# HKU-MedAI/WSI-HGNN

Hardware: AMD Instinct MI355X
Metric: edges/s fwd+bwd HEATNet4, 10k-node/6-rel synth graph, 1->8 MI355X (higher is better)
Workload: dtype f32 (fp16x3 emulation: 2-way fp16 split scaled per row (Y = XW^T, dX) or per column (dW), 3 products - bf16x6 for small launches; fp32-class error)

## Files before the change

### include/wsi_hgnn.h

```cpp
#ifndef WSI_HGNN_H
#define WSI_HGNN_H

#include <stdint.h>

#ifdef __cplusplus
extern "C" {
#endif

#define WSI_OK        0
#define WSI_EINVAL  (-22)
#define WSI_ENOSYS  (-38)
#define WSI_EFAULT  (-14)
#define WSI_ENOMEM  (-12)

#define WSI_ABI_VERSION 26

int         wsi_abi_version(void);
const char* wsi_last_error(void);

typedef struct wsi_context wsi_context_t;
int  wsi_context_create(wsi_context_t** out);
void wsi_context_destroy(wsi_context_t* ctx);

#define WSI_ATTN_XCD_CONTIGUOUS 1
#define WSI_ATTN_HUB_DEGREE(d) (((d) & 0xffff) << 8)
int wsi_heat_attn_fwd(const float* q, int64_t ldq, const float* k, int64_t ldk, const float* v, int64_t ldv,
                      int32_t num_nodes, int32_t D, int32_t H,
                      const int32_t* node_seg, const int32_t* rowptr, const int32_t* src, const float* sim,
                      const int32_t* order, int32_t num_heavy, int32_t flags,
                      const float* e_weight, const float* e_bias,
                      float* t, int64_t ldt, float* score, float* lse,
                      uint32_t* t_absmax,
                      wsi_context_t* ctx, void* stream);

int wsi_heat_attn_scores_fwd(const float* q, int64_t ldq, const float* k, int64_t ldk, int32_t num_nodes, int32_t D, int32_t H,
                             const int32_t* node_seg, const int32_t* rowptr, const int32_t* src, const float* sim,
                             const int32_t* order, int32_t num_heavy, int32_t flags, const float* e_weight, const float* e_bias,
                             float* score, float* lse, wsi_context_t* ctx, void* stream);

int wsi_heat_pool_coeff(const float* score, const float* lse, const int32_t* edge_seg,
                        const int32_t* colptr, const int32_t* csc_eid, const int32_t* csc_dst, const float* inv_rd,
                        const int32_t* row_seg, int32_t segs_per_type, int32_t n_types, int32_t H, int32_t num_src,
                        float* ctab, void* stream);

int wsi_heat_pool_gtab(const float* h, int64_t ldh, int32_t D, int32_t H, const float* y, const float* beta,
                       const int32_t* chunk_row, const int32_t* chunk_seg, int32_t num_chunks,
                       int32_t segs_per_type, int32_t n_types, float* gtab, void* stream);

typedef struct wsi_attn_pool {
    const int32_t* row_seg;
    int32_t segs_per_type, n_types;
    const float* y;
    const float* g_row;
    const float* omg;
    float* r_out; int64_t ldr;
    float* ctab;
    int32_t ctab_ready;
    const float* h; int64_t ldh;
    const float* beta;
    const float* gtab;
    const int32_t* edge_seg;
    const int32_t* seg_dst;
} wsi_attn_pool_t;

int wsi_heat_attn_bwd(const float* q, int64_t ldq, const float* k, int64_t ldk, const float* v, int64_t ldv,
                      int32_t num_nodes, int32_t num_src, int32_t num_edges, int32_t D, int32_t H,
                      const int32_t* node_seg, const int32_t* rowptr, const int32_t* src, const float* sim,
                      const int32_t* colptr, const int32_t* csc_eid, const int32_t* csc_dst,
                      const float* inv_rd, const int32_t* order_dst, int32_t num_heavy, const int32_t* order_src, int32_t flags,
                      const float* e_weight, const float* e_bias,
                      const float* g_t, int64_t ldgt,
                      const int32_t* g_t_row,
                      const float* score,
                      float* score_a,
                      const float* lse,
                      float* ga, float* gsc, float* gea, float* red_ws,
                      float* gq, int64_t ldgq, float* gk, int64_t ldgk, float* gv, int64_t ldgv,
                      float* g_e,
                      uint32_t* g_absmax,
                      const wsi_attn_pool_t* pool,
                      wsi_context_t* ctx, void* stream);

typedef struct wsi_gemm_group {
    const float* A;
    const float* B;
    float*       C;
    const float* bias;
    const float* R;
    const float* gate;
    const float* B1;
    const float* B2;
    int64_t lda, ldb, ldc, ldr;
    int32_t M, N, K;
    int32_t b_chunk;
    const float* Mm;
    int64_t  ldm;
    float*   colsum_out;
    const uint32_t* a_absmax;
    uint32_t*       c_absmax;
    int32_t a_absmax_parts;
    int32_t c_absmax_parts;
    int32_t c_absmax_first;
    int32_t reserved;
    uint32_t drop_seed;
    uint32_t drop_threshold;
    float    drop_scale;
    int32_t  drop_row0;
    int32_t  drop_cols;
    int32_t  drop_col0;
    const uint32_t* drop_seed_base;
    uint32_t*       c_colmax;
    float*          c_colsum;
    int64_t         c_col_ld;
    const uint32_t* a_colmax;
    const float*    a_colsum;
    const uint32_t* b_colmax;
    int64_t         a_col_ld, b_col_ld;
    int32_t         a_col_parts, b_col_parts;
    void*           b_packed;
} wsi_gemm_group_t;

#define WSI_GEMM_NT 0
#define WSI_GEMM_NN 1
#define WSI_GEMM_TN 2

#define WSI_EPI_BIAS        1
#define WSI_EPI_ACCUMULATE  2
#define WSI_EPI_SCALE_GATE  4
#define WSI_EPI_GELU        8
#define WSI_EPI_ADD_R       16
// ... 222 lines not shown
```

### wsi-hgnn_amd/csrc/gemm_tn16.hip

```cpp
#include "gemm_common.h"
#include "emu16.h"

namespace wsi {

typedef __attribute__((__vector_size__(4 * sizeof(__fp16)))) __fp16 h16x4;
typedef __attribute__((address_space(3))) h16x4 lds_h16x4;
typedef _Float16 f16x4 __attribute__((ext_vector_type(4)));

constexpr int T_M = 256;
constexpr int T_THREADS = 512;
constexpr int T_KS = 16;
#ifndef T_NS_DEF
#define T_NS_DEF 3
#endif
constexpr int T_NS = T_NS_DEF;
constexpr int T_CH = 256;

struct TnGroup {
    const float* A; const float* B;
    const uint32_t* abits; const uint32_t* bbits;
    int64_t lda, ldb;
    int64_t ws_off;
    int32_t M, N, K;
    int32_t tile_start, tiles_n, tiles_mn, kchunk, flags;
};
struct TnParams {
    TnGroup g[WSI_GEMM_MAX_GROUPS];
    int32_t ngroups, total_tiles;
};

__device__ __forceinline__ f16x8 tr_read8(const uint16_t* p0, const uint16_t* p1) {
    const h16x4 lo = __builtin_amdgcn_ds_read_tr16_b64_v4f16((lds_h16x4*)p0);
    const h16x4 hi = __builtin_amdgcn_ds_read_tr16_b64_v4f16((lds_h16x4*)p1);
    const f16x4 a = __builtin_bit_cast(f16x4, lo), b = __builtin_bit_cast(f16x4, hi);
    return __builtin_shufflevector(a, b, 0, 1, 2, 3, 4, 5, 6, 7);
}

template <int TN_, int NACC>
__global__ __launch_bounds__(T_THREADS, 2) void gemm_tn16_kernel(const TnParams P, float* __restrict__ ws) {
    static_assert(TN_ == 128 || TN_ == 256, "tile width");
    constexpr int PA = T_M + 32, PB = TN_ + 32;
    constexpr int PLANE_A = T_KS * PA, PLANE_B = T_KS * PB;
    constexpr int BUF = 2 * (PLANE_A + PLANE_B);
    constexpr int CB = TN_ / 4;
    constexpr int NBQ = TN_ / 128;
    constexpr int RB = T_THREADS / CB;
    constexpr int WTN = TN_ / 64;
    __shared__ __attribute__((aligned(16))) uint16_t smem[2 * BUF];

    const int tid = threadIdx.x;
    const int tile = xcd_remap((int)blockIdx.x, P.total_tiles);
    int gi = 0;
#pragma unroll 1
    for (int i = 1; i < P.ngroups; ++i) gi = (tile >= P.g[i].tile_start) ? i : gi;
    const TnGroup& G = P.g[gi];
    int local = tile - G.tile_start;
    const int split = local / G.tiles_mn;
    local -= split * G.tiles_mn;
    const int tm = local / G.tiles_n, tn = local - tm * G.tiles_n;
    const int m0 = tm * T_M, n0 = tn * TN_;
    const int kb = split * G.kchunk, ke = min(G.K, kb + G.kchunk);
    const int lane = tid & 63, wave = tid >> 6;
    const int wm = wave >> 1, wn = wave & 1;
    const int l31 = lane & 31, hi = lane >> 5;

    const int c4a = tid & 63, ra = tid >> 6;
    const int c4b = tid % CB, rb = tid / CB;
    float sa[4], sb[4];
#pragma unroll
    for (int i = 0; i < 4; ++i) {
        sa[i] = __builtin_ldexpf(1.f, -scale_exponent(G.abits[min(m0 + 4 * c4a + i, G.M - 1)]));
        sb[i] = __builtin_ldexpf(1.f, -scale_exponent(G.bbits[min(n0 + 4 * c4b + i, G.N - 1)]));
    }
    const int wA = min(T_M, G.M - m0), wB = min(TN_, G.N - n0);
    const bool fast = (G.flags & 1) && (G.flags & 2) && (wA % 4 == 0) && (wB % 4 == 0) && ke > kb &&
                      (int64_t)(ke - kb) * G.lda * 4 < ((int64_t)1 << 31) && (int64_t)(ke - kb) * G.ldb * 4 < ((int64_t)1 << 31);
    typedef uint32_t u32x4 __attribute__((ext_vector_type(4)));
    const float* baseA = G.A + (int64_t)kb * G.lda + m0;
    const float* baseB = G.B + (int64_t)kb * G.ldb + n0;
    const auto rsA = __builtin_amdgcn_make_buffer_rsrc(const_cast<float*>(baseA), 0, fast ? (int)(((int64_t)(ke - kb - 1) * G.lda + wA) * 4) : 0, 0x00020000);
    const auto rsB = __builtin_amdgcn_make_buffer_rsrc(const_cast<float*>(baseB), 0, fast ? (int)(((int64_t)(ke - kb - 1) * G.ldb + wB) * 4) : 0, 0x00020000);
    const int voA = (int)((ra * G.lda + 4 * c4a) * 4), voB = (int)((rb * G.ldb + 4 * c4b) * 4);
    const int stepA = (int)(G.lda * 4), stepB = (int)(G.ldb * 4);
    struct Stage { float4 a[2]; float4 b[NBQ]; };
    auto as_f4 = [](const u32x4& v) { return make_float4(__uint_as_float(v[0]), __uint_as_float(v[1]), __uint_as_float(v[2]), __uint_as_float(v[3])); };
    auto load_fast = [&](Stage& S, int s) {
#pragma unroll
        for (int q = 0; q < 2; ++q) S.a[q] = as_f4(__builtin_amdgcn_raw_buffer_load_b128(rsA, voA, (s * T_KS + 8 * q) * stepA, 0));
#pragma unroll
        for (int q = 0; q < NBQ; ++q) S.b[q] = as_f4(__builtin_amdgcn_raw_buffer_load_b128(rsB, voB, (s * T_KS + RB * q) * stepB, 0));
    };
    auto load4g = [](const float* __restrict__ row, int c0, int c_end) {
        float4 r = make_float4(0.f, 0.f, 0.f, 0.f);
        if (c0 + 0 < c_end) r.x = row[c0 + 0];
        if (c0 + 1 < c_end) r.y = row[c0 + 1];
        if (c0 + 2 < c_end) r.z = row[c0 + 2];
        if (c0 + 3 < c_end) r.w = row[c0 + 3];
        return r;
    };
    auto load_guarded = [&](Stage& S, int k0) {
#pragma unroll
        for (int q = 0; q < 2; ++q) {
            const int k = k0 + ra + 8 * q;
            S.a[q] = (k < ke) ? load4g(G.A + (int64_t)k * G.lda, m0 + 4 * c4a, G.M) : make_float4(0.f, 0.f, 0.f, 0.f);
        }
#pragma unroll
        for (int q = 0; q < NBQ; ++q) {
            const int k = k0 + rb + RB * q;
            S.b[q] = (k < ke) ? load4g(G.B + (int64_t)k * G.ldb, n0 + 4 * c4b, G.N) : make_float4(0.f, 0.f, 0.f, 0.f);
        }
    };
    const int nfast = fast ? (ke - kb + T_KS - 1) / T_KS : 0;
// ... 50 lines not shown
#pragma unroll
        for (int i = 0; i < 2; ++i)
#pragma unroll
            for (int j = 0; j < WTN; ++j) c[i][j] = __builtin_amdgcn_mfma_f32_32x32x16_f16(a[i], b[j], c[i][j], 0, 0, 0);
    };
    constexpr int CX = NACC - 1;
    auto multiply_stage = [&](const uint16_t* buf) {
        f16x8 a0[2], a1[2], b0[WTN], b1[WTN];
        read_a(buf, 0, a0);
        read_b(buf, 1, b1);
        read_a(buf, 1, a1);
        read_b(buf, 0, b0);
        products(acc[CX], a0, b1);
        products(acc[CX], a1, b0);
        products(acc[0], a0, b0);
    };

    if (nfast > 0) {
        constexpr int NS = (TN_ == 128) ? T_NS : 2;
        Stage R[NS];
        struct Frags { f16x8 a0[2], a1[2], b0[WTN], b1[WTN]; };
        auto body = [&](Frags& c, Frags& n, Stage& C, Stage& F, int s) {
            load_fast(F, min(s + NS, nfast - 1));
            const uint16_t* cur = smem + (s & 1) * BUF;
            uint16_t* oth = smem + ((s + 1) & 1) * BUF;
            __builtin_amdgcn_s_setprio(2);
            read_a(cur, 1, c.a1);
            read_b(cur, 0, c.b0);
            products(acc[CX], c.a0, c.b1);
            store_stage(C, oth);
            products(acc[CX], c.a1, c.b0);
            __builtin_amdgcn_sched_group_barrier(0x020, 2 + NBQ, 0);
            __builtin_amdgcn_sched_group_barrier(0x100, 2 * (2 + WTN), 0);
#pragma unroll
            for (int m = 0; m < 4 * WTN; ++m) {
                __builtin_amdgcn_sched_group_barrier(0x008, 1, 0);
                __builtin_amdgcn_sched_group_barrier(0x002, 3, 0);
                if (m >= 4 * WTN - (2 + NBQ)) __builtin_amdgcn_sched_group_barrier(0x200, 2, 0);
            }
            __builtin_amdgcn_s_setprio(0);
            __builtin_amdgcn_sched_barrier(0);
            __syncthreads();
            read_a(oth, 0, n.a0);
            read_b(oth, 1, n.b1);
            products(acc[0], c.a0, c.b0);
            __builtin_amdgcn_sched_barrier(0);
        };
#pragma unroll
        for (int q = 0; q < NS; ++q) load_fast(R[q], min(q, nfast - 1));
        store_stage(R[0], smem);
        __syncthreads();
        Frags X, Y;
        read_a(smem, 0, X.a0);
        read_b(smem, 1, X.b1);
        int s = 0;
        for (; s + 2 * NS <= nfast; s += 2 * NS) {
#pragma unroll
            for (int q = 0; q < 2 * NS; ++q) {
                if (q & 1) body(Y, X, R[(q + 1) % NS], R[q % NS], s + q);
                else body(X, Y, R[(q + 1) % NS], R[q % NS], s + q);
            }
        }
#pragma unroll
        for (int q = 0; q < 2 * NS - 1; ++q) {
            if (s + q < nfast) {
                if (q & 1) body(Y, X, R[(q + 1) % NS], R[q % NS], s + q);
                else body(X, Y, R[(q + 1) % NS], R[q % NS], s + q);
            }
        }
    }
    for (int k0 = kb + nfast * T_KS; k0 < ke; k0 += T_KS) {
        Stage g;
        load_guarded(g, k0);
        store_stage(g, smem);
        __syncthreads();
        multiply_stage(smem);
        __syncthreads();
    }

    int* se = reinterpret_cast<int*>(smem);
    for (int i = tid; i < T_M + TN_; i += T_THREADS)
        se[i] = (i < T_M) ? scale_exponent(G.abits[min(m0 + i, G.M - 1)]) : scale_exponent(G.bbits[min(n0 + i - T_M, G.N - 1)]);
    __syncthreads();
    float* slab = ws + G.ws_off + (int64_t)split * G.M * G.N;
#pragma unroll
    for (int j = 0; j < WTN; ++j) {
        const int cl = wn * (TN_ / 2) + j * 32 + l31;
        const int col = n0 + cl;
        const int ec = se[T_M + cl];
#pragma unroll
        for (int i = 0; i < 2; ++i)
#pragma unroll
            for (int r = 0; r < 16; ++r) {
                const int rl = wm * 64 + i * 32 + (r & 3) + 8 * (r >> 2) + 4 * hi;
                const int row = m0 + rl;
                float x = acc[0][i][j][r];
                if constexpr (NACC == 2) x = fmaf(acc[1][i][j][r], 1.f / LO_SCALE, x);
                x = __builtin_ldexpf(x, ec + se[rl]);
                if (row < G.M && col < G.N) slab[(int64_t)row * G.N + col] = x;
            }
    }
}

struct ColJob {
    const float* X; int64_t ld;
    const uint32_t* part;
    const float* psum;
    int64_t part_ld;
    int32_t own;
    uint32_t* out;
    float* sum_out;
    const float* gate;
    int32_t rows, cols, cols_pad, chunks, col_blocks;
    int32_t block_start;
    int32_t fblock_start;
    int32_t vec;
};
struct ColParams {
    ColJob j[2 * WSI_GEMM_MAX_GROUPS];
    int32_t njobs, epilogue;
};

__global__ __launch_bounds__(256) void colstat_partial_kernel(const ColParams P) {
    __shared__ float4 sm[256], ss[256];
    int ji = 0;
#pragma unroll 1
    for (int i = 1; i < P.njobs; ++i) ji = (P.j[i].own && (int)blockIdx.x >= P.j[i].block_start) ? i : ji;
    const ColJob& J = P.j[ji];
    if (!J.own) return;
    const int b = (int)blockIdx.x - J.block_start;
    const int chunk = b / J.col_blocks, cb = b - chunk * J.col_blocks;
    const int c4 = threadIdx.x & 63, rl = threadIdx.x >> 6;
    const int c0 = cb * 256 + 4 * c4;
    const int r0 = chunk * T_CH, r1 = min(J.rows, r0 + T_CH);
    float4 m = make_float4(0.f, 0.f, 0.f, 0.f), t = make_float4(0.f, 0.f, 0.f, 0.f);
    if (J.vec && c0 + 3 < J.cols) {
        const float* p = J.X + c0;
#pragma unroll 4
        for (int r = r0 + rl; r < r1; r += 4) {
            const float4 v = *reinterpret_cast<const float4*>(p + (int64_t)r * J.ld);
            m.x = fmaxf(m.x, fabsf(v.x)); m.y = fmaxf(m.y, fabsf(v.y)); m.z = fmaxf(m.z, fabsf(v.z)); m.w = fmaxf(m.w, fabsf(v.w));
            t.x += v.x; t.y += v.y; t.z += v.z; t.w += v.w;
        }
    } else if (c0 < J.cols) {
        for (int r = r0 + rl; r < r1; r += 4) {
            const float* p = J.X + (int64_t)r * J.ld + c0;
            m.x = fmaxf(m.x, fabsf(p[0])); t.x += p[0];
            if (c0 + 1 < J.cols) { m.y = fmaxf(m.y, fabsf(p[1])); t.y += p[1]; }
            if (c0 + 2 < J.cols) { m.z = fmaxf(m.z, fabsf(p[2])); t.z += p[2]; }
            if (c0 + 3 < J.cols) { m.w = fmaxf(m.w, fabsf(p[3])); t.w += p[3]; }
        }
    }
    sm[threadIdx.x] = m;
    ss[threadIdx.x] = t;
    __syncthreads();
    if (rl == 0 && c0 < J.cols_pad) {
#pragma unroll
        for (int q = 1; q < 4; ++q) {
            const float4 o = sm[c4 + 64 * q], u = ss[c4 + 64 * q];
            m.x = fmaxf(m.x, o.x); m.y = fmaxf(m.y, o.y); m.z = fmaxf(m.z, o.z); m.w = fmaxf(m.w, o.w);
            t.x += u.x; t.y += u.y; t.z += u.z; t.w += u.w;
        }
        *reinterpret_cast<uint4*>(const_cast<uint32_t*>(J.part) + (int64_t)chunk * J.part_ld + c0) =
            make_uint4(__float_as_uint(m.x), __float_as_uint(m.y), __float_as_uint(m.z), __float_as_uint(m.w));
        if (J.psum) *reinterpret_cast<float4*>(const_cast<float*>(J.psum) + (int64_t)chunk * J.part_ld + c0) = t;
    }
}

constexpr int CF_COLS = 16, CF_LANES = 256 / CF_COLS;
__global__ __launch_bounds__(256) void colstat_final_kernel(const ColParams P) {
    __shared__ uint32_t sm[256];
    __shared__ float ss[256];
    int ji = 0;
#pragma unroll 1
    for (int i = 1; i < P.njobs; ++i) ji = ((int)blockIdx.x >= P.j[i].fblock_start) ? i : ji;
    const ColJob& J = P.j[ji];
    const int cl = threadIdx.x % CF_COLS, kl = threadIdx.x / CF_COLS;
    const int c = ((int)blockIdx.x - J.fblock_start) * CF_COLS + cl;
    uint32_t m = 0u;
    float t = 0.f;
    if (c < J.cols) {
        const uint32_t* pm = J.part + c;
// ... 31 lines not shown

static inline bool tn_vec_ok(const void* p, int64_t ld) { return ((reinterpret_cast<uintptr_t>(p) & 15) == 0) && (ld % 4 == 0); }

static int tn16_tile_n() {
    const char* s = knob("WSI_TN16_CFG");
    return (s && s[0] == '2') ? 256 : 128;
}

struct Tn16Plan {
    int32_t splits[WSI_GEMM_MAX_GROUPS];
    int32_t kchunk[WSI_GEMM_MAX_GROUPS];
    int32_t tiles_m[WSI_GEMM_MAX_GROUPS], tiles_n[WSI_GEMM_MAX_GROUPS];
    int32_t total_tiles;
};

static void tn16_plan(const wsi_gemm_group_t* g, int32_t ng, int tn, Tn16Plan& pl) {
    const int64_t target = 256;
    int64_t work = 0, maxk = 0;
    for (int i = 0; i < ng; ++i) {
        pl.tiles_m[i] = pl.tiles_n[i] = 0; pl.splits[i] = 1; pl.kchunk[i] = g[i].K > 0 ? g[i].K : T_KS;
        if (g[i].M <= 0 || g[i].N <= 0) continue;
        pl.tiles_m[i] = (g[i].M + T_M - 1) / T_M; pl.tiles_n[i] = (g[i].N + tn - 1) / tn;
        work += (int64_t)pl.tiles_m[i] * pl.tiles_n[i] * g[i].K;
        if (g[i].K > maxk) maxk = g[i].K;
    }
    int64_t kc = (work + target - 1) / target;
    kc = ((kc + T_KS - 1) / T_KS) * T_KS;
    if (kc < 8 * T_KS) kc = 8 * T_KS;
    for (;;) {
        int64_t blocks = 0;
        for (int i = 0; i < ng; ++i) {
            if (!pl.tiles_m[i]) continue;
            pl.splits[i] = g[i].K > 0 ? (int32_t)((g[i].K + kc - 1) / kc) : 1;
            blocks += (int64_t)pl.tiles_m[i] * pl.tiles_n[i] * pl.splits[i];
        }
        if (blocks <= target || kc >= maxk) break;
        kc += T_KS;
    }
    int32_t tiles = 0;
    for (int i = 0; i < ng; ++i) {
        if (!pl.tiles_m[i]) continue;
        if (g[i].K > 0) {
            int64_t per = (g[i].K + pl.splits[i] - 1) / pl.splits[i];
            per = ((per + T_KS - 1) / T_KS) * T_KS;
            pl.kchunk[i] = (int32_t)per;
            pl.splits[i] = (int32_t)((g[i].K + per - 1) / per);
        }
        tiles += pl.tiles_m[i] * pl.tiles_n[i] * pl.splits[i];
    }
    pl.total_tiles = tiles;
}

static inline int64_t pad4(int64_t x) { return (x + 3) & ~(int64_t)3; }

int64_t tn16_workspace_floats(const wsi_gemm_group_t* groups, int32_t ngroups) {
    Tn16Plan pl;
    tn16_plan(groups, ngroups, tn16_tile_n(), pl);
    int64_t f = 0;
    for (int i = 0; i < ngroups; ++i) {
        if (groups[i].M <= 0 || groups[i].N <= 0) continue;
        f += (int64_t)pl.splits[i] * groups[i].M * groups[i].N;
    }
    f = pad4(f);
    for (int i = 0; i < ngroups; ++i) {
        if (groups[i].M <= 0 || groups[i].N <= 0) continue;
        const int64_t chunks = (groups[i].K + T_CH - 1) / T_CH;
        f += (pad4(groups[i].M) + pad4(groups[i].N)) * (1 + chunks) + (groups[i].colsum_out ? pad4(groups[i].M) * chunks : 0);
    }
    return f;
}

int launch_gemm_tn16(int32_t epilogue, const wsi_gemm_group_t* groups, int32_t ngroups, float* ws, int64_t ws_bytes, hipStream_t st) {
    const int tn = tn16_tile_n();
    Tn16Plan pl;
    tn16_plan(groups, ngroups, tn, pl);
    const int64_t need = tn16_workspace_floats(groups, ngroups);
    if (need >= ((int64_t)1 << 31)) { set_error("gemm TN fp16x3: workspace of %lld floats exceeds the 2^31 index range", (long long)need); return WSI_EINVAL; }
    if (!ws || ws_bytes < need * 4) { set_error("gemm TN fp16x3: workspace of %lld bytes needed, %lld given", (long long)(need * 4), (long long)ws_bytes); return WSI_ENOMEM; }
    if (reinterpret_cast<uintptr_t>(ws) & 15) { set_error("gemm TN fp16x3: the workspace must be 16-byte aligned"); return WSI_EINVAL; }
    TnParams P;
    ReduceParams RP;
    ColParams CP;
    P.ngroups = 0; RP.ngroups = 0; RP.epilogue = epilogue; CP.njobs = 0;
    int64_t f = 0, red_total = 0;
    int32_t tiles = 0;
    for (int i = 0; i < ngroups; ++i) {
        const wsi_gemm_group_t& s = groups[i];
        if (s.M <= 0 || s.N <= 0) continue;
        TnGroup& d = P.g[P.ngroups];
        d.A = s.A; d.B = s.B; d.lda = s.lda; d.ldb = s.ldb; d.M = s.M; d.N = s.N; d.K = s.K;
        d.tiles_n = pl.tiles_n[i]; d.tiles_mn = pl.tiles_m[i] * pl.tiles_n[i]; d.kchunk = pl.kchunk[i];
        d.tile_start = tiles;
        tiles += d.tiles_mn * pl.splits[i];
        d.flags = (tn_vec_ok(s.A, s.lda) ? 1 : 0) | (tn_vec_ok(s.B, s.ldb) ? 2 : 0);
        d.ws_off = f;
        ReduceDesc& r = RP.g[RP.ngroups++];
        r.ws = ws + f; r.C = s.C; r.gate = s.gate; r.ldc = s.ldc; r.M = s.M; r.N = s.N; r.pad = 0; r.splits = pl.splits[i]; r.start = red_total;
        red_total += (int64_t)s.M * s.N;
        f += (int64_t)pl.splits[i] * s.M * s.N;
        r.cs_ws = nullptr; r.cs_out = nullptr;
        P.ngroups++;
    }
    if (P.ngroups == 0) return WSI_OK;
    P.total_tiles = tiles;
    f = pad4(f);
    uint32_t* wu = reinterpret_cast<uint32_t*>(ws);
    int32_t pblocks = 0, fblocks = 0;
    CP.epilogue = epilogue;
    auto job_for = [&](const float* X, int64_t ld, int32_t rows, int32_t cols, float* sum_out, const float* gate,
                       const uint32_t* gmax, const float* gsum, int64_t gld, int32_t gparts, int64_t& cursor) -> const uint32_t* {
        if (gmax && (gparts < 1 || (sum_out && !gsum))) gmax = nullptr;
        for (int q = 0; q < CP.njobs; ++q) {
            ColJob& J = CP.j[q];
            if (J.X == X && J.ld == ld && J.rows == rows && J.cols == cols && !sum_out && (J.own || J.part == gmax)) return J.out;
        }
        ColJob& J = CP.j[CP.njobs++];
        J.X = X; J.ld = ld; J.rows = rows; J.cols = cols; J.cols_pad = (int32_t)pad4(cols);
        J.col_blocks = (cols + 255) / 256;
        J.out = wu + cursor; cursor += J.cols_pad;
        J.sum_out = sum_out; J.gate = gate;
        if (gmax) {
            J.own = 0; J.part = gmax; J.psum = sum_out ? gsum : nullptr; J.part_ld = gld; J.chunks = gparts; J.vec = 0;
            J.block_start = pblocks;
        } else {
            J.own = 1; J.part_ld = J.cols_pad; J.chunks = (rows + T_CH - 1) / T_CH;
            J.part = wu + cursor; cursor += (int64_t)J.chunks * J.cols_pad;
            J.psum = nullptr;
            if (sum_out) { J.psum = reinterpret_cast<float*>(wu + cursor); cursor += (int64_t)J.chunks * J.cols_pad; }
            J.vec = tn_vec_ok(X, ld) ? 1 : 0;
            J.block_start = pblocks; pblocks += J.chunks * J.col_blocks;
        }
        J.fblock_start = fblocks; fblocks += (cols + CF_COLS - 1) / CF_COLS;
        return J.out;
    };
    {
        int gidx = 0;
        for (int i = 0; i < ngroups; ++i) {
            const wsi_gemm_group_t& s = groups[i];
            if (s.M <= 0 || s.N <= 0) continue;
            TnGroup& d = P.g[gidx++];
            int64_t cursor = f;
            d.abits = job_for(s.A, s.lda, s.K, s.M, s.colsum_out, s.gate, s.a_colmax, s.a_colsum, s.a_col_ld, s.a_col_parts, cursor);
            d.bbits = job_for(s.B, s.ldb, s.K, s.N, nullptr, nullptr, s.b_colmax, nullptr, s.b_col_ld, s.b_col_parts, cursor);
            const int64_t chunks = (s.K + T_CH - 1) / T_CH;
            f += (pad4(s.M) + pad4(s.N)) * (1 + chunks) + (s.colsum_out ? pad4(s.M) * chunks : 0);
        }
    }
    if (pblocks > 0) hipLaunchKernelGGL(colstat_partial_kernel, dim3(pblocks), dim3(256), 0, st, CP);
    hipLaunchKernelGGL(colstat_final_kernel, dim3(fblocks), dim3(256), 0, st, CP);
#ifdef WSI_ABLATE
    if (tn == 256) hipLaunchKernelGGL((gemm_tn16_kernel<256, 1>), dim3(tiles), dim3(T_THREADS), 0, st, P, ws);
    else
#endif
    hipLaunchKernelGGL((gemm_tn16_kernel<128, 2>), dim3(tiles), dim3(T_THREADS), 0, st, P, ws);
    RP.total = red_total;
    launch_splitk_reduce(RP, st);
    return check_launch("gemm_tn16");
}

}

using namespace wsi;

extern "C" int32_t wsi_col_stats_parts(int32_t rows) { return rows > 0 ? (rows + T_CH - 1) / T_CH : 0; }

extern "C" int wsi_col_stats(const float* x, int64_t ld, int32_t rows, int32_t cols, uint32_t* part_max, float* part_sum, int64_t part_ld, void* stream) {
    if (rows < 0 || cols < 0) { set_error("col_stats: bad shape %d x %d", rows, cols); return WSI_EINVAL; }
    if (rows == 0 || cols == 0) return WSI_OK;
    if (!x || !part_max || part_ld < ((cols + 3) & ~3) || (part_ld & 3) || (reinterpret_cast<uintptr_t>(part_max) & 15) || (part_sum && (reinterpret_cast<uintptr_t>(part_sum) & 15))) {
        set_error("col_stats: null pointer, or tables not 16-byte aligned with a pitch >= the columns rounded up to 4"); return WSI_EINVAL; }
    ColParams CP;
    CP.njobs = 1; CP.epilogue = 0;
    ColJob& J = CP.j[0];
    J.X = x; J.ld = ld; J.rows = rows; J.cols = cols; J.cols_pad = (int32_t)pad4(cols); J.col_blocks = (cols + 255) / 256;
    J.out = nullptr; J.sum_out = nullptr; J.gate = nullptr; J.own = 1; J.part_ld = part_ld; J.chunks = (rows + T_CH - 1) / T_CH;
    J.part = part_max; J.psum = part_sum; J.vec = tn_vec_ok(x, ld) ? 1 : 0;
    J.block_start = 0; J.fblock_start = 0;
    hipLaunchKernelGGL(colstat_partial_kernel, dim3(J.chunks * J.col_blocks), dim3(256), 0, (hipStream_t)stream, CP);
    return check_launch("col_stats");
}

extern "C" int64_t wsi_col_absmax_workspace_bytes(int32_t rows, int32_t cols) {
    if (rows <= 0 || cols <= 0) return 0;
    return (int64_t)((rows + T_CH - 1) / T_CH) * pad4(cols) * 4;
}

extern "C" int wsi_col_absmax(const float* x, int64_t ld, int32_t rows, int32_t cols, uint32_t* out, void* workspace, int64_t workspace_bytes, void* stream) {
    if (rows < 0 || cols < 0) { set_error("col_absmax: bad shape %d x %d", rows, cols); return WSI_EINVAL; }
    if (cols == 0) return WSI_OK;
    if (!out || (rows > 0 && !x)) { set_error("col_absmax: null pointer"); return WSI_EINVAL; }
    const int64_t need = wsi_col_absmax_workspace_bytes(rows, cols);
    if (need > 0 && (!workspace || workspace_bytes < need || (reinterpret_cast<uintptr_t>(workspace) & 15))) {
        set_error("col_absmax: a 16-byte aligned workspace of %lld bytes is needed", (long long)need); return WSI_ENOMEM; }
    ColParams CP;
    CP.njobs = 1; CP.epilogue = 0;
    ColJob& J = CP.j[0];
    J.X = x; J.ld = ld; J.rows = rows; J.cols = cols; J.cols_pad = (int32_t)pad4(cols); J.col_blocks = (cols + 255) / 256;
    J.out = out; J.sum_out = nullptr; J.gate = nullptr; J.own = 1; J.part_ld = J.cols_pad; J.chunks = (rows + T_CH - 1) / T_CH;
    J.part = reinterpret_cast<uint32_t*>(workspace); J.psum = nullptr; J.vec = tn_vec_ok(x, ld) ? 1 : 0;
    J.block_start = 0; J.fblock_start = 0;
    hipStream_t st = (hipStream_t)stream;
    if (J.chunks > 0) hipLaunchKernelGGL(colstat_partial_kernel, dim3(J.chunks * J.col_blocks), dim3(256), 0, st, CP);
    hipLaunchKernelGGL(colstat_final_kernel, dim3((cols + CF_COLS - 1) / CF_COLS), dim3(256), 0, st, CP);
    return check_launch("col_absmax");
}
```

### wsi-hgnn_amd/csrc/loss.hip

```cpp
#include "common.h"
#include <math.h>

namespace wsi {

constexpr int64_t CE_IGNORE_INDEX = -100;
__global__ __launch_bounds__(256) void cross_entropy_kernel(const float* __restrict__ logits, const int64_t* __restrict__ labels, int B, int C,
                                                            float* __restrict__ loss, float* __restrict__ dlogits, int* __restrict__ bad) {
    __shared__ float part[256];
    __shared__ int cnt[256];
    __shared__ int any_bad;
    if (threadIdx.x == 0) any_bad = 0;
    int valid = 0;
    for (int b = threadIdx.x; b < B; b += 256) {
        const int64_t y = labels[b];
        valid += (y >= 0 && y < C) ? 1 : 0;
    }
    cnt[threadIdx.x] = valid;
    __syncthreads();
    for (int o = 128; o > 0; o >>= 1) {
        if ((int)threadIdx.x < o) cnt[threadIdx.x] += cnt[threadIdx.x + o];
        __syncthreads();
    }
    const int nvalid = cnt[0];
    const float invB = nvalid > 0 ? 1.f / (float)nvalid : 0.f;
    float acc = 0.f;
    for (int b = threadIdx.x; b < B; b += 256) {
        const float* row = logits + (int64_t)b * C;
        const int64_t y = labels[b];
        if (y < 0 || y >= C) {
            if (y != CE_IGNORE_INDEX) { any_bad = 1; if (bad) *bad = 1; }
            for (int c = 0; c < C; ++c) dlogits[(int64_t)b * C + c] = 0.f;
            continue;
        }
        float mx = -INFINITY;
        for (int c = 0; c < C; ++c) mx = fmaxf(mx, row[c]);
        float den = 0.f;
        for (int c = 0; c < C; ++c) den += expf(row[c] - mx);
        acc += (logf(den) + mx) - row[y];
        const float inv = 1.f / den;
        for (int c = 0; c < C; ++c) dlogits[(int64_t)b * C + c] = (expf(row[c] - mx) * inv - (c == y ? 1.f : 0.f)) * invB;
    }
    part[threadIdx.x] = acc;
    __syncthreads();
    for (int o = 128; o > 0; o >>= 1) {
        if ((int)threadIdx.x < o) part[threadIdx.x] += part[threadIdx.x + o];
        __syncthreads();
    }
    if (threadIdx.x == 0) *loss = any_bad ? NAN : part[0] / (float)nvalid;
}

}

using namespace wsi;

extern "C" int wsi_cross_entropy(const float* logits, const int64_t* labels, int32_t B, int32_t C, float* loss, float* dlogits, int32_t* bad_label,
                                 void* stream) {
    if (B <= 0 || C <= 0 || (int64_t)B * C > 65536) { set_error("cross_entropy: unsupported shape %d x %d", B, C); return WSI_ENOSYS; }
    if (!logits || !labels || !loss || !dlogits) { set_error("cross_entropy: null pointer"); return WSI_EINVAL; }
    hipLaunchKernelGGL(cross_entropy_kernel, dim3(1), dim3(256), 0, (hipStream_t)stream, logits, labels, (int)B, (int)C, loss, dlogits, (int*)bad_label);
    return check_launch("cross_entropy");
}
```

### wsi-hgnn_amd/ops.py

```python
from __future__ import annotations

import ctypes
import contextlib
from typing import List, Optional, Sequence, Tuple

import torch

from . import _native as N
from .graph import GraphPlan, SegmentTable, host_to_device



_TIMING = {"on": False, "records": []}


def enable_kernel_timing(on: bool) -> None:
    _TIMING["on"] = bool(on)
    _TIMING["records"] = []


class _Timed:
    def __init__(self, name: str, flops: float = 0.0, mfma_flops: float = 0.0):
        self.name, self.flops, self.mfma_flops = name, flops, mfma_flops

# ... 196 lines not shown
        st = _SIDE_STREAMS["streams"][key] = torch.cuda.Stream(device=dev)
    return st


def _side_stats_on() -> bool:
    return _SIDE_STATS["enabled"] and not _SIDE_STATS["reasons"] and not torch.cuda.is_current_stream_capturing()


def block_side_streams(blocked: bool, who: str) -> None:
    (_SIDE_STATS["reasons"].add if blocked else _SIDE_STATS["reasons"].discard)(who)
    block_background_weight_gradients(blocked, who=who)


def set_side_column_statistics(on: bool) -> None:
    _SIDE_STATS["enabled"] = bool(on)


def _col_stats_side(x: torch.Tensor, rows: Sequence[Tuple[int, int]], device):
    if not _side_stats_on():
        return None
    lib = N.load()
    dev = torch.device(device)
    width = x.shape[1]
    wpad = (width + 3) & ~3
    ranges, p = {}, 0
    for (a, b) in rows:
        if (a, b) not in ranges and b > a:
            n_ = lib.wsi_col_stats_parts(b - a)
            ranges[(a, b)] = (p, n_)
            p += n_
    if p == 0:
        return None
    bits = torch.empty((p, wpad), dtype=torch.int32, device=dev)
    sums = torch.empty((p, wpad), dtype=torch.float32, device=dev)
    side = side_stream(dev, "stats")
    main = torch.cuda.current_stream(dev)
    side.wait_stream(main)
    for (a, b), (p0, n_) in ranges.items():
        N.check(lib.wsi_col_stats(N.ptr(x, a * x.stride(0) * 4), x.stride(0), b - a, width, N.ptr(bits, p0 * wpad * 4), N.ptr(sums, p0 * wpad * 4), wpad,
                                  ctypes.c_void_p(side.cuda_stream)), "wsi_col_stats")
        _SIDE_STATS["launches"] += 1
    ev = torch.cuda.Event()
    ev.record(side)
    for t_ in (x, bits, sums):
        t_.record_stream(side)
    return ColStats(bits, sums, ranges), ev


def remember_constant_cols(x: torch.Tensor, rows: Sequence[Tuple[int, int]]) -> None:
    if _PRECISION["mode"] not in _SCALED_MODES or x.dim() != 2 or not x.is_cuda or x.stride(1) != 1:
        return
    st = _annotation(x, "_wsi_col_stats")
    if st is not None and all(r in st.ranges for r in rows if r[1] > r[0]):
        return
    lib = N.load()
    width = x.shape[1]
    ranges, bits_rows = {}, []
    for (a, b) in rows:
        if (a, b) in ranges or b <= a:
            continue
        out = torch.empty(width, dtype=torch.int32, device=x.device)
        nbytes = lib.wsi_col_absmax_workspace_bytes(b - a, width)
        ws = torch.empty(max(nbytes // 4, 4), dtype=torch.int32, device=x.device)
        N.check(lib.wsi_col_absmax(N.ptr(x, a * x.stride(0) * 4), x.stride(0), b - a, width, N.ptr(out), N.ptr(ws), nbytes, N.stream()), "wsi_col_absmax")
        ranges[(a, b)] = (len(bits_rows), 1)
        bits_rows.append(out)
    if bits_rows:
        attach_col_stats(x, ColStats(torch.stack(bits_rows), None, ranges))


def refresh_constant_cols(x: torch.Tensor) -> None:
    st = _annotation(x, "_wsi_col_stats")
    if st is None or st.sums is not None:
        return
    lib = N.load()
    width = x.shape[1]
    for (a, b), (p0, _) in st.ranges.items():
        nbytes = lib.wsi_col_absmax_workspace_bytes(b - a, width)
        ws = torch.empty(max(nbytes // 4, 4), dtype=torch.int32, device=x.device)
        N.check(lib.wsi_col_absmax(N.ptr(x, a * x.stride(0) * 4), x.stride(0), b - a, width, N.ptr(st.bits, p0 * st.bits.shape[1] * 4), N.ptr(ws), nbytes,
                                   N.stream()), "wsi_col_absmax")


_PACKED = {"enabled": True, "entries": {}, "hits": 0, "packs": 0}


def set_packed_weight_cache(on: bool) -> None:
    _PACKED["enabled"] = bool(on)
    if not on:
        _PACKED["entries"].clear()


def invalidate_packed_weights() -> None:
    _PACKED["entries"].clear()


def _pack_groups(op: int, items, arm: bool) -> None:
    lib = N.load()
    for i in range(0, len(items), N.WSI_GEMM_MAX_GROUPS):
        chunk = items[i:i + N.WSI_GEMM_MAX_GROUPS]
        arr = _group_array([g for _, g in chunk])
        N.check(lib.wsi_gemm_pack_b(op, arr, len(chunk), N.stream()), "wsi_gemm_pack_b")
        _PACKED["packs"] += 1
        for e, _ in chunk:
            e["versions"] = tuple(w._version for w in e["weights"])
            e["armed"] = arm


def _attach_packed(op: int, chunk: Sequence[dict], arr) -> None:
    import weakref
    ent = _PACKED["entries"]
    for gi, g in enumerate(chunk):
        ws_ = g.get("Bw")
        if not ws_ or any(not isinstance(w, torch.nn.Parameter) for w in ws_):
            continue
        key = (op, tuple(w.data_ptr() for w in ws_), g["N"], g["K"], g.get("b_chunk", 0), g["ldb"])
        e = ent.get(key)
        if e is not None and any(r() is not w for r, w in zip(e["refs"], ws_)):
            e = None
        if e is None:
            if len(ent) >= 256:
                dead = [k_ for k_, e_ in ent.items() if any(r() is None for r in e_["refs"])]
                for k_ in dead:
                    ent.pop(k_)
                if len(ent) >= 256:
                    ent.pop(next(iter(ent)))
            nbytes = N.load().wsi_gemm_packed_b_bytes(g["N"], g["K"])
            e = ent[key] = {"buf": torch.empty(nbytes // 4, dtype=torch.int32, device=ws_[0].device), "refs": [weakref.ref(w) for w in ws_],
                            "weights": None, "versions": None, "op": op, "armed": False,
                            "group": dict(B=g["B"], B1=g.get("B1"), B2=g.get("B2"), ldb=g["ldb"], N=g["N"], K=g["K"], b_chunk=g.get("b_chunk", 0))}
            e["group"]["b_packed"] = N.ptr(e["buf"])
            continue
        if e["armed"] and e["versions"] == tuple(w._version for w in ws_):
            _PACKED["hits"] += 1
            e["armed"] = False
            arr[gi].b_packed = e["group"]["b_packed"]


def repack_weights() -> None:
    if not _PACKED["enabled"] or not _PACKED["entries"] or torch.cuda.is_current_stream_capturing():
        return
    by_op = {}
    dead = []
    for key, e in _PACKED["entries"].items():
        ws_ = [r() for r in e["refs"]]
        if any(w is None for w in ws_):
            dead.append(key)
            continue
        e["weights"] = ws_
        by_op.setdefault(e["op"], []).append((e, e["group"]))
    for key in dead:
        _PACKED["entries"].pop(key, None)
    for op, items in by_op.items():
        _pack_groups(op, items, arm=True)
    for e in _PACKED["entries"].values():
        e["weights"] = None


def _gemm(op: int, epilogue: int, groups: Sequence[dict], device) -> bool:
    lib = N.load()
    prec = _GEMM_MODES[_PRECISION["mode"]]
    groups = [g for g in groups if g["M"] > 0 and g["N"] > 0]
    wrote = True
    for i in range(0, len(groups), N.WSI_GEMM_MAX_GROUPS):
        chunk = groups[i:i + N.WSI_GEMM_MAX_GROUPS]
        arr = _group_array(chunk)
        if any(g.get("c_colmax") for g in chunk):
            wrote = wrote and bool(lib.wsi_gemm_writes_colstats(op, prec, arr, len(chunk)))
        ws = None
        ws_bytes = 0
        kernel = lib.wsi_gemm_kernel_precision(op, prec, arr, len(chunk))
        if kernel == N.WSI_GEMM_FP16X3 and op != N.WSI_GEMM_TN and _PACKED["enabled"] and not torch.cuda.is_current_stream_capturing():
            _attach_packed(op, chunk, arr)
        if op == N.WSI_GEMM_TN or kernel == N.WSI_GEMM_FP16X3:
            ws_bytes = lib.wsi_gemm_workspace_bytes(op, prec, arr, len(chunk))
            ws = torch.empty(max(ws_bytes // 4, 1), dtype=torch.float32, device=device)
        if not _TIMING["on"]:
            N.check(lib.wsi_gemm_grouped(op, epilogue, prec, arr, len(chunk), N.ptr(ws), ws_bytes, N.stream()), "wsi_gemm_grouped")
            continue
        flops = sum(2.0 * g["M"] * g["N"] * g["K"] for g in chunk)
        products = {N.WSI_GEMM_FP32: 1.0, N.WSI_GEMM_BF16X6: 6.0, N.WSI_GEMM_FP16X3: 3.0}[kernel]
        with _Timed("gemm", flops, flops * products), _Timed(("gemm_nt", "gemm_nn", "gemm_tn")[op] + ("_fp32", "_bf16x6", "_fp16x3")[kernel], flops, flops * products):
            N.check(lib.wsi_gemm_grouped(op, epilogue, prec, arr, len(chunk), N.ptr(ws), ws_bytes, N.stream()), "wsi_gemm_grouped")
    return wrote


_GROUP_FIELDS = [f[0] for f in N.GemmGroup._fields_]
_GROUP_INDEX = {name: i for i, name in enumerate(_GROUP_FIELDS)}
_GROUP_DEFAULT = tuple(1.0 if name == "drop_scale" else (None if N.GemmGroup._fields_[i][1] is ctypes.c_void_p else 0) for i, name in enumerate(_GROUP_FIELDS))


def _group_array(chunk):
    index, default = _GROUP_INDEX, _GROUP_DEFAULT
    rows = []
    for g in chunk:
        vals = list(default)
        for k, v in g.items():
            i = index.get(k)
            if i is not None:
                vals[i] = v
        rows.append(N.GemmGroup(*vals))
    return (N.GemmGroup * len(rows))(*rows)


_SMALL_PAIR = {"enabled": True}


def _gemm_small_pair(dx_groups: Sequence[dict], dx_epilogue: int, dw_groups: Sequence[dict], dw_epilogue: int, device) -> bool:
    dx_groups = [g for g in dx_groups if g["M"] > 0 and g["N"] > 0]
    dw_groups = [g for g in dw_groups if g["M"] > 0 and g["N"] > 0]
    if (not _SMALL_PAIR["enabled"] or not dx_groups or not dw_groups or len(dx_groups) + len(dw_groups) > 16
            or any(g["M"] > 32 or g.get("c_absmax") or g.get("b_chunk") for g in dx_groups) or any(g["K"] > 32 or g.get("c_absmax") for g in dw_groups)):
        return False
    flops = sum(2.0 * g["M"] * g["N"] * g["K"] for g in list(dx_groups) + list(dw_groups))
    with _Timed("gemm", flops, flops), _Timed("gemm_small_pair", flops, flops):
        N.check(N.load().wsi_gemm_small_pair(_group_array(dx_groups), len(dx_groups), dx_epilogue, _group_array(dw_groups), len(dw_groups), dw_epilogue,
                                             N.stream()), "wsi_gemm_small_pair")
    return True


_BACKGROUND = {"enabled": True, "min_flop": 3.0e10, "queued": [], "pending": [], "armed": False, "blocked": False,
               "launches": 0, "task": -1, "written": set()}


def set_background_weight_gradients(on: bool) -> None:
    _BACKGROUND["enabled"] = bool(on)


def block_background_weight_gradients(blocked: bool, who: str = "bucket") -> None:
    reasons = _BACKGROUND.setdefault("reasons", set())
    (reasons.add if blocked else reasons.discard)(who)
    _BACKGROUND["blocked"] = bool(reasons)


def _background_flush(device, to_side: bool = True) -> None:
    st = _BACKGROUND
    if not st["queued"]:
# ... 1211 lines not shown
                                       **_scale_in(gkqv_max, r0), **_scale_out(gh_max, r0),
                                       **(gh_cols.produce(r0, r1, 0) if gh_cols is not None else {})))
                gh_wrote = _gemm(N.WSI_GEMM_NN, epi, groups, dev) and gh_wrote
            else:
                for j in range(3):
                    groups = []
                    for i in idxs:
                        r0, r1 = hctx.rows[i]
                        groups.append(dict(A=N.ptr(gkqv, (r0 * 3 * D + blk[j] * D) * 4), lda=3 * D, B=N.ptr(P[i][j]), ldb=D,
                                           C=N.ptr(g_h, r0 * D * 4), ldc=D, R=N.ptr(g_out, r0 * D * 4), ldr=D,
                                           gate=gate(i) if with_gate else None, M=r1 - r0, N=D, K=D))
                    _gemm(N.WSI_GEMM_NN, epi if j == 0 else N.WSI_EPI_ACCUMULATE, groups, dev)
        wgroups = []
        h_cols = getattr(ctx, "h_cols", None)
        for i, (r0, r1) in enumerate(hctx.rows):
            for j in range(nproj):
                gw = torch.empty_like(P[i][j])
                gb = torch.empty_like(P[i][4 + j])
                grads[8 * i + j] = gw
                grads[8 * i + 4 + j] = gb
                wgroups.append(dict(A=N.ptr(gkqv, (r0 * ldp + blk[j] * D) * 4), lda=ldp, B=N.ptr(h, r0 * D * 4), ldb=D,
                                    C=N.ptr(gw), ldc=D, colsum_out=N.ptr(gb), M=D, N=D, K=r1 - r0,
                                    **(gk_side[0].consume("a", r0, r1, blk[j] * D, want_sums=True) if gk_side is not None else {}),
                                    **(h_cols.consume("b", r0, r1, 0) if h_cols is not None else {})))
        wr = [P[i][k] for i in range(T) for j in range(nproj) for k in (j, 4 + j)]
        keep = [gkqv, h] + ([h_cols.bits] if h_cols is not None else []) + ([gk_side[0].bits, gk_side[0].sums] if gk_side is not None else [])
        outs = [(P[i][k], grads[8 * i + k]) for i in range(T) for j in range(nproj) for k in (j, 4 + j)]
        evs = [gk_side[1]] if gk_side is not None else []
        if not (ctx.background_dw and _background_safe(wr) and _gemm_tn_background(0, wgroups, dev, keep, wr, evs, outs=outs)):
            for ev in evs:
                torch.cuda.current_stream(dev).wait_event(ev)
            _gemm(N.WSI_GEMM_TN, 0, wgroups, dev)
        if collapse:
            if not no_v:
                hp, csum = _pooled_factors(h, ctab, bc.rp, T, H)
                N.check(lib.wsi_pool_bwd_bias(N.ptr(gt_seg), T, S, D, H, None, N.ptr(csum), None, N.ptr(gbv), N.stream()), "wsi_pool_bwd_bias")
            wgroups = []
            for tau in range(T):
                gw = torch.empty_like(P[tau][2])
                grads[8 * tau + 2] = gw
                grads[8 * tau + 6] = gbv[tau]
                for hh in range(H):
                    wgroups.append(dict(A=N.ptr(gt_seg, hh * dk * 4), lda=D, B=N.ptr(hp, (hh * T + tau) * D * 4), ldb=H * T * D,
                                        C=N.ptr(gw, hh * dk * D * 4), ldc=D, M=dk, N=D, K=S))
            _gemm(N.WSI_GEMM_TN, 0, wgroups, dev)
        if gh_max is not None and chunked:
            attach_row_scales(g_h, gh_max)
        if gh_cols is not None and gh_wrote and chunked:
            attach_col_stats(g_h, gh_cols)
        if early_gate is not None:
            torch.cuda.current_stream(dev).wait_event(early_gate[1])
        return (g_h, None, None, g_skip, g_e[0:1].view(1, 1), g_e[1:2], None, None, None, *grads)


def heat_layer_fused(h, hctx, H, skip, e_weight, e_bias, params, drop_mask=None, pool=None, background_dw=False):
    if pool is not None:
        pool = (pool[0], {"sum": N.WSI_RED_SUM, "mean": N.WSI_RED_MEAN}[pool[1]])
    return _HeatLayerFused.apply(h, hctx, H, skip, e_weight, e_bias, drop_mask, pool, background_dw, *params)


class _CrossEntropy(torch.autograd.Function):

    @staticmethod
    def forward(ctx, logits, labels, bad):
        N.require_cuda(logits, labels)
        logits = logits.contiguous()
        labels = labels.contiguous()
        if labels.dtype != torch.int64 or logits.dim() != 2 or labels.shape != logits.shape[:1]:
            raise ValueError("cross_entropy: logits [B, C] fp32 and int64 labels [B]")
        B, C = logits.shape
        out = torch.empty(1 + B * C, dtype=torch.float32, device=logits.device)
        N.check(N.load().wsi_cross_entropy(N.ptr(logits), N.ptr(labels), B, C, N.ptr(out), N.ptr(out, 4), N.ptr(bad), N.stream()), "wsi_cross_entropy")
        ctx.save_for_backward(out)
        ctx.shape = (B, C)
        return out[0]

    @staticmethod
    def backward(ctx, g):
        (out,) = ctx.saved_tensors
        return out[1:].view(ctx.shape) * g, None, None


def cross_entropy(logits: torch.Tensor, labels: torch.Tensor) -> torch.Tensor:
    bad = torch.zeros(1, dtype=torch.int32, device=logits.device)
    loss = _CrossEntropy.apply(logits, labels, bad)
    loss._wsi_bad_label = bad
    return loss


class _RelationAttention(torch.autograd.Function):

    @staticmethod
    def forward(ctx, q, kv, e_weight, e_bias, plan: GraphPlan, sim_csr, D: int, H: int):
        N.require_cuda(q, kv)
        lib = N.load()
        q = q.contiguous()
        kv = kv.contiguous()
        n, E, S = plan.num_nodes, plan.num_edges, plan.num_segs
        dev = q.device
        t = torch.empty((n, D), dtype=torch.float32, device=dev)
        score = torch.empty((max(E, 1), H), dtype=torch.float32, device=dev)
        lse = torch.empty((max(S, 1), H), dtype=torch.float32, device=dev)
        ew, eb = e_weight.reshape(-1), e_bias.reshape(-1)
        with _Timed("heat_attn"):
            N.check(lib.wsi_heat_attn_fwd(
                N.ptr(q), q.stride(0), N.ptr(kv, 0), kv.stride(0), N.ptr(kv, D * 4), kv.stride(0), n, D, H,
                N.ptr(plan.node_seg), N.ptr(plan.rowptr), N.ptr(plan.src), N.ptr(sim_csr), N.ptr(plan.order_dst), plan.num_heavy, _attn_flags(plan),
                N.ptr(ew), N.ptr(eb), N.ptr(t), D, N.ptr(score), N.ptr(lse), None, N.context(), N.stream()), "wsi_heat_attn_fwd")
        ctx.plan, ctx.D, ctx.H = plan, D, H
        ctx.save_for_backward(q, kv, ew, eb, sim_csr, score, lse)
        return t

    @staticmethod
    def backward(ctx, g_t):
        lib = N.load()
        plan, D, H = ctx.plan, ctx.D, ctx.H
        q, kv, ew, eb, sim_csr, score, lse = ctx.saved_tensors
        g_t = g_t.contiguous()
        n, E = plan.num_nodes, plan.num_edges
        dev = q.device
        a = torch.empty_like(score)
        scratch = torch.empty((3, max(E, 1), H), dtype=torch.float32, device=dev)
        red_ws = torch.empty(1024, dtype=torch.float32, device=dev)
        gq = torch.empty_like(q)
        gkv = torch.empty_like(kv)
        g_e = torch.empty(2, dtype=torch.float32, device=dev)
        with _Timed("heat_attn"):
            N.check(lib.wsi_heat_attn_bwd(
                N.ptr(q), q.stride(0), N.ptr(kv, 0), kv.stride(0), N.ptr(kv, D * 4), kv.stride(0),
                n, plan.num_src_rows, E, D, H,
                N.ptr(plan.node_seg), N.ptr(plan.rowptr), N.ptr(plan.src), N.ptr(sim_csr),
                N.ptr(plan.colptr), N.ptr(plan.csc_eid), N.ptr(plan.csc_dst),
                N.ptr(plan.inv_rd), N.ptr(plan.order_dst), plan.num_heavy, N.ptr(plan.order_src), _attn_flags(plan), N.ptr(ew), N.ptr(eb),
                N.ptr(g_t), g_t.stride(0), None, N.ptr(score), N.ptr(a), N.ptr(lse), N.ptr(scratch[0]), N.ptr(scratch[1]), N.ptr(scratch[2]), N.ptr(red_ws),
                N.ptr(gq), gq.stride(0), N.ptr(gkv, 0), gkv.stride(0), N.ptr(gkv, D * 4), gkv.stride(0),
                N.ptr(g_e), None, None, N.context(), N.stream()), "wsi_heat_attn_bwd")
        return gq, gkv, g_e[0:1].view(1, 1), g_e[1:2], None, None, None, None


def relation_attention(q, kv, e_weight, e_bias, plan: GraphPlan, sim_csr, D: int, H: int) -> torch.Tensor:
    return _RelationAttention.apply(q, kv, e_weight, e_bias, plan, sim_csr, D, H)


class _GatedLinear(torch.autograd.Function):
    @staticmethod
    def forward(ctx, t, h, skip, rows, nids, rplan, seg_of, n_g, drop_mask, *params):
        N.require_cuda(t, h)
        t = t.contiguous()
        h = h.contiguous()
        dev = t.device
        n, D = h.shape
        K = t.shape[1]
        ws, bs = params[:n_g], params[n_g:]
        covered = sum(b - a for a, b in rows) == n
        z = torch.empty((n, D), dtype=torch.float32, device=dev) if covered else h.clone()
        groups = []
        for i, (r0, r1) in enumerate(rows):
            groups.append(dict(A=N.ptr(t, r0 * K * 4), lda=K, B=N.ptr(ws[i]), ldb=K, C=N.ptr(z, r0 * D * 4), ldc=D,
                               bias=N.ptr(bs[i]), R=N.ptr(h, r0 * D * 4), ldr=D, gate=N.ptr(skip, 4 * nids[i]),
                               Mm=N.ptr(drop_mask, r0 * D * 4) if drop_mask is not None else None, ldm=D,
                               M=r1 - r0, N=D, K=K))
        _gemm(N.WSI_GEMM_NT, N.WSI_EPI_GATED_SKIP | (N.WSI_EPI_MUL_M if drop_mask is not None else 0), groups, dev)
        ctx.rows, ctx.nids, ctx.rplan, ctx.seg_of, ctx.n_g, ctx.covered = rows, nids, rplan, seg_of, n_g, covered
        ctx.has_mask = drop_mask is not None
        ctx.save_for_backward(t, h, z, skip, *(() if drop_mask is None else (drop_mask,)), *ws)
        return z

# ... 644 lines not shown
```

Before: 112.3 million.

## Write TN GEMM output directly when unsplit, pack weights on side stream

When no group uses split-K, the fp16x3 TN GEMM kernel now applies the gate and accumulate epilogue itself and stores straight to C, so the separate split-K reduce launch and the workspace round trip are skipped. NN weight repacking is moved onto a side stream, with an event that the consumer waits on before it uses the packed buffer. The cross-entropy bad-label flag is now zeroed inside the kernel instead of by a separate torch.zeros fill. These changes remove launches and serial work at the cost of extra stream and event bookkeeping.

```diff
diff --git a/include/wsi_hgnn.h b/include/wsi_hgnn.h
--- a/include/wsi_hgnn.h
+++ b/include/wsi_hgnn.h
@@ -46,6 +46,7 @@
 int wsi_heat_pool_gtab(const float* h, int64_t ldh, int32_t D, int32_t H, const float* y, const float* beta,
                        const int32_t* chunk_row, const int32_t* chunk_seg, int32_t num_chunks,
                        int32_t segs_per_type, int32_t n_types, float* gtab, void* stream);
+
 
 typedef struct wsi_attn_pool {
     const int32_t* row_seg;
diff --git a/wsi-hgnn_amd/csrc/gemm_tn16.hip b/wsi-hgnn_amd/csrc/gemm_tn16.hip
--- a/wsi-hgnn_amd/csrc/gemm_tn16.hip
+++ b/wsi-hgnn_amd/csrc/gemm_tn16.hip
@@ -23,11 +23,22 @@
     int64_t ws_off;
     int32_t M, N, K;
     int32_t tile_start, tiles_n, tiles_mn, kchunk, flags;
+    float* C; const float* gate; int64_t ldc;
 };
 struct TnParams {
     TnGroup g[WSI_GEMM_MAX_GROUPS];
     int32_t ngroups, total_tiles;
+    int32_t direct, epilogue;
 };
+
+__device__ __forceinline__ float tn_gate_factor(int32_t epilogue, const float* gate) {
+    return ((epilogue & WSI_EPI_SCALE_GATE) && gate) ? 1.f / (1.f + expf(-(*gate))) : 1.f;
+}
+__device__ __forceinline__ float tn_finish_value(float s, int32_t epilogue, bool gated, float gs, const float* c) {
+    if (gated) s = __fmul_rn(s, gs);
+    if (epilogue & WSI_EPI_ACCUMULATE) s = __fadd_rn(s, *c);
+    return s;
+}
 
 __device__ __forceinline__ f16x8 tr_read8(const uint16_t* p0, const uint16_t* p1) {
     const h16x4 lo = __builtin_amdgcn_ds_read_tr16_b64_v4f16((lds_h16x4*)p0);
@@ -244,7 +255,11 @@
     for (int i = tid; i < T_M + TN_; i += T_THREADS)
         se[i] = (i < T_M) ? scale_exponent(G.abits[min(m0 + i, G.M - 1)]) : scale_exponent(G.bbits[min(n0 + i - T_M, G.N - 1)]);
     __syncthreads();
-    float* slab = ws + G.ws_off + (int64_t)split * G.M * G.N;
+    const bool direct = P.direct != 0;
+    const bool gated = (P.epilogue & WSI_EPI_SCALE_GATE) && G.gate;
+    const float gs = direct ? tn_gate_factor(P.epilogue, G.gate) : 1.f;
+    const int64_t mn = (int64_t)G.M * G.N;
+    float* slab = ws + G.ws_off + (int64_t)split * mn;
 #pragma unroll
     for (int j = 0; j < WTN; ++j) {
         const int cl = wn * (TN_ / 2) + j * 32 + l31;
@@ -259,7 +274,12 @@
                 float x = acc[0][i][j][r];
                 if constexpr (NACC == 2) x = fmaf(acc[1][i][j][r], 1.f / LO_SCALE, x);
                 x = __builtin_ldexpf(x, ec + se[rl]);
-                if (row < G.M && col < G.N) slab[(int64_t)row * G.N + col] = x;
+                if (row < G.M && col < G.N) {
+                    if (direct) {
+                        float* c = G.C + (int64_t)row * G.ldc + col;
+                        *c = tn_finish_value(__fadd_rn(0.f, x), P.epilogue, gated, gs, c);
+                    } else slab[(int64_t)row * G.N + col] = x;
+                }
             }
     }
 }
@@ -457,6 +477,11 @@
     ReduceParams RP;
     ColParams CP;
     P.ngroups = 0; RP.ngroups = 0; RP.epilogue = epilogue; CP.njobs = 0;
+    const char* two = knob("WSI_TN_REDUCE");
+    bool direct = !(two && two[0] == '2');
+    for (int i = 0; i < ngroups; ++i) direct = direct && (groups[i].M <= 0 || groups[i].N <= 0 || pl.splits[i] == 1);
+    P.direct = direct ? 1 : 0;
+    P.epilogue = epilogue;
     int64_t f = 0, red_total = 0;
     int32_t tiles = 0;
     for (int i = 0; i < ngroups; ++i) {
@@ -469,6 +494,7 @@
         tiles += d.tiles_mn * pl.splits[i];
         d.flags = (tn_vec_ok(s.A, s.lda) ? 1 : 0) | (tn_vec_ok(s.B, s.ldb) ? 2 : 0);
         d.ws_off = f;
+        d.C = s.C; d.gate = s.gate; d.ldc = s.ldc;
         ReduceDesc& r = RP.g[RP.ngroups++];
         r.ws = ws + f; r.C = s.C; r.gate = s.gate; r.ldc = s.ldc; r.M = s.M; r.N = s.N; r.pad = 0; r.splits = pl.splits[i]; r.start = red_total;
         red_total += (int64_t)s.M * s.N;
@@ -528,8 +554,10 @@
     else
 #endif
     hipLaunchKernelGGL((gemm_tn16_kernel<128, 2>), dim3(tiles), dim3(T_THREADS), 0, st, P, ws);
-    RP.total = red_total;
-    launch_splitk_reduce(RP, st);
+    if (!P.direct) {
+        RP.total = red_total;
+        launch_splitk_reduce(RP, st);
+    }
     return check_launch("gemm_tn16");
 }
 
diff --git a/wsi-hgnn_amd/csrc/loss.hip b/wsi-hgnn_amd/csrc/loss.hip
--- a/wsi-hgnn_amd/csrc/loss.hip
+++ b/wsi-hgnn_amd/csrc/loss.hip
@@ -9,7 +9,10 @@
     __shared__ float part[256];
     __shared__ int cnt[256];
     __shared__ int any_bad;
-    if (threadIdx.x == 0) any_bad = 0;
+    if (threadIdx.x == 0) {
+        any_bad = 0;
+        if (bad) *bad = 0;
+    }
     int valid = 0;
     for (int b = threadIdx.x; b < B; b += 256) {
         const int64_t y = labels[b];
diff --git a/wsi-hgnn_amd/ops.py b/wsi-hgnn_amd/ops.py
--- a/wsi-hgnn_amd/ops.py
+++ b/wsi-hgnn_amd/ops.py
@@ -302,13 +302,17 @@
                                    N.stream()), "wsi_col_absmax")
 
 
-_PACKED = {"enabled": True, "entries": {}, "hits": 0, "packs": 0}
+_PACKED = {"enabled": True, "entries": {}, "hits": 0, "packs": 0, "side": True}
 
 
 def set_packed_weight_cache(on: bool) -> None:
     _PACKED["enabled"] = bool(on)
     if not on:
         _PACKED["entries"].clear()
+
+
+def set_side_weight_pack(on: bool) -> None:
+    _PACKED["side"] = bool(on)
 
 
 def invalidate_packed_weights() -> None:
@@ -354,6 +358,10 @@
         if e["armed"] and e["versions"] == tuple(w._version for w in ws_):
             _PACKED["hits"] += 1
             e["armed"] = False
+            ev = e.get("ready")
+            if ev is not None:
+                torch.cuda.current_stream(e["buf"].device).wait_event(ev)
+                e["ready"] = None
             arr[gi].b_packed = e["group"]["b_packed"]
 
 
@@ -372,7 +380,21 @@
     for key in dead:
         _PACKED["entries"].pop(key, None)
     for op, items in by_op.items():
-        _pack_groups(op, items, arm=True)
+        if op == N.WSI_GEMM_NN and _PACKED["side"] and not _SIDE_STATS["reasons"]:
+            dev = items[0][0]["buf"].device
+            st = side_stream(dev)
+            st.wait_stream(torch.cuda.current_stream(dev))
+            with torch.cuda.stream(st):
+                _pack_groups(op, items, arm=True)
+            ev = torch.cuda.Event()
+            ev.record(st)
+            for e, _ in items:
+                e["buf"].record_stream(st)
+                e["ready"] = ev
+        else:
+            _pack_groups(op, items, arm=True)
+            for e, _ in items:
+                e["ready"] = None
     for e in _PACKED["entries"].values():
         e["weights"] = None
 
@@ -1750,7 +1772,7 @@
 
 
 def cross_entropy(logits: torch.Tensor, labels: torch.Tensor) -> torch.Tensor:
-    bad = torch.zeros(1, dtype=torch.int32, device=logits.device)
+    bad = torch.empty(1, dtype=torch.int32, device=logits.device)
     loss = _CrossEntropy.apply(logits, labels, bad)
     loss._wsi_bad_label = bad
     return loss
```

Result: no change. 112.2 million (-0.1%).
